# gafniguy/4D-Facial-Avatars

Measured on AMD Instinct MI355X. Metric: rays/sec at 512x512, 64 coarse + 128 fine samples, higher is better.
Workload: dtype f32; 1 GPU; configs[1]: paper-model eval forward, 512x512 frame, 64+128 samples, chunksize 65536, perturb on, expression+latent conditioned, background prior; frames sharded over GPUs

## Files before the change

### 4d-facial-avatars_amd/csrc/nf_mlp_gated.hip

```cpp
#include "nf_mlp_live_kernel.h"

__global__ void __launch_bounds__(256) k_paper_sigma_bound(const float* __restrict__ packed, float* __restrict__ bound) {
    using Net = NfPaperNet;
    __shared__ double sw[16][16], sv[16][16], sc[16], sd[16];
    __shared__ float fw[16], fv[16];
    const int tid = threadIdx.x, ni = blockIdx.x, part = tid >> 4, kk = tid & 15;
    auto alpha = [&](int n) { return (double)packed[Net::OFF_D0 + (((n >> 4) * 9 + 8) * 64 + ((n >> 2) & 3) * 16) * 4 + (n & 3)]; };
    double w = 0.0, v = 0.0, c = 0.0, d = 0.0;
    for (int j = 0; j < 16; ++j) {
        const int n = 16 * part + j;
        const double a = alpha(n);
        const double f = (double)packed[Net::OFF_FEAT + ((ni * 16 + (n >> 4)) * 64 + (kk >> 2) * 16 + (n & 15)) * 4 + (kk & 3)];
        w += a * f;
        v += fabs(a) * fabs(f);
        if (ni == 0 && kk == 0) {
            const double b = (double)packed[Net::OFF_BIAS + Net::B_FEAT + n];
            c += a * b;
            d += fabs(a) * fabs(b);
        }
    }
    sw[part][kk] = w;
    sv[part][kk] = v;
    if (kk == 0) {
        sc[part] = c;
        sd[part] = d;
    }
    __syncthreads();
    auto up = [](double x) {
        float f = (float)x;
        if ((double)f < x) f = nextafterf(f, INFINITY);
        return f;
    };
    if (tid < 16) {
        double tw = 0.0, tv = 0.0;
        for (int q = 0; q < 16; ++q) {
            tw += sw[q][tid];
            tv += sv[q][tid];
        }
        fw[tid] = (float)tw;
        fv[tid] = up(tv);
    }
    if (ni == 0 && tid == 16) {
        const double b = (double)packed[Net::OFF_BIAS + Net::B_D0 + 128];
        double tc = 0.0, td = 0.0;
        for (int q = 0; q < 16; ++q) {
            tc += sc[q];
            td += sd[q];
        }
        for (int j = 0; j < 16; ++j) bound[NF_BOUND_BIAS + j] = j == 0 ? (float)(tc + b) : (j == 1 ? up(td + fabs(b)) : 0.0f);
    }
    __syncthreads();
    const int lane = tid >> 2, r = tid & 3, g = lane >> 4, i = lane & 15;
    bound[(ni * 64 + lane) * 4 + r] = i == 0 ? fw[4 * g + r] : (i == 1 ? fv[4 * g + r] : 0.0f);
}

extern "C" size_t nf_paper_sigma_bound_floats(void) { return NF_BOUND_FLOATS; }

extern "C" int nf_paper_sigma_bound(const float* packed, float* bound, nf_stream_t stream) {
    if (!packed || !bound || ((uintptr_t)bound & 15)) return NF_EINVAL;
    hipLaunchKernelGGL(k_paper_sigma_bound, dim3(16), dim3(256), 0, nf_s(stream), packed, bound);
    NF_RETURN_LAUNCH();
}

extern "C" int nf_paper_mlp_fwd_gated(const float* packed, const float* bound, const float* cond, const float* ro, const float* rd,
                                      const float* rd_view, const float* z, int64_t n_rays, int n_samples, float* raw, float* scratch,
                                      size_t scratch_floats, int max_workgroups, nf_stream_t stream) {
    return nf_live_launch<false, true>(packed, cond, ro, rd, rd_view, z, n_rays, n_samples, raw, scratch, scratch_floats, max_workgroups, nullptr,
                                       stream, bound);
}
```

### 4d-facial-avatars_amd/csrc/nf_mlp_live_kernel.h

```cpp
#pragma once
#include <mutex>
#include "nf_mlp_paper_net.h"

#define NF_LIVE_ROWS 64
#ifndef NF_LIVE_PF
#define NF_LIVE_PF 8
#endif
#define NF_LIVE_DIR_B (NF_LIVE_ROWS * 1024)
#define NF_LIVE_META_B (NF_LIVE_DIR_B + NF_LIVE_ROWS * 64)
#define NF_LIVE_WAVE_B (NF_LIVE_META_B + NF_LIVE_ROWS * 16)
#define NF_LIVE_OOB NF_LIVE_WAVE_B
#define NF_LIVE_SC1 16

static_assert(NF_LIVE_ROWS == 64 && NF_MLP_NT == 2, "row numbers wrap with & 63; a pass's liveness is one 32-bit mask");
static_assert(NF_LIVE_PF >= 0 && NF_LIVE_PF <= 16, "prefetched rows live in registers beside fc_alpha's weights");

__device__ __forceinline__ __amdgpu_buffer_rsrc_t nf_live_ring(char* ring_v) {
    const uint64_t a = (uint64_t)ring_v;
    const uint64_t s = (uint64_t)(uint32_t)__builtin_amdgcn_readfirstlane((int)(uint32_t)a) |
                       ((uint64_t)(uint32_t)__builtin_amdgcn_readfirstlane((int)(a >> 32)) << 32);
    return __builtin_amdgcn_make_buffer_rsrc(reinterpret_cast<char*>(s), (short)0, NF_LIVE_WAVE_B, 0x00020000);
}
__device__ __forceinline__ void nf_live_store(__amdgpu_buffer_rsrc_t ring, int off_b, f32x4 v) {
    __builtin_amdgcn_raw_buffer_store_b128(__builtin_bit_cast(nf_u32x4, v), ring, off_b, 0, 0);
// ... 252 lines not shown
                    }
                }
                head_v = head + n_live;
                asm volatile("" : "+v"(head_v));
            }
            nf_live_mark<STATS, COLS>(stats, NF_LIVE_PH_APPEND, -1);
        } else {
            if constexpr (GATE) {
                NfGatePre pre{st, pf, ring_v, head_v, tail_v, bound_v};
                pre.wait();
                pre.loads(Wi, Ci, lane);
            } else {
                NfLivePre pre{st, wd, pf, ring_v, head_v, tail_v};
                pre.wait();
                pre.loads(Wi, Ci, lane);
            }
#pragma unroll
            for (int t = 0; t < NT; ++t) {
                dirf[t][0] = (f32x4){0.0f, 0.0f, 0.0f, 0.0f};
                sigma_own[t] = 0.0f;
            }
            run_v = __builtin_amdgcn_readfirstlane(head_v) != __builtin_amdgcn_readfirstlane(tail_v) ? 2 : 0;
        }
        asm volatile("" : "+v"(live_v), "+v"(run_v));
        const int run = __builtin_amdgcn_readfirstlane(run_v);
        if (run != 0) {
            nf_live_stat<STATS, COLS>(stats, NF_LIVE_STAT_RUNS, 1);
            if (run == 2) nf_live_stat<STATS, COLS>(stats, NF_LIVE_STAT_FLUSH, __builtin_amdgcn_readfirstlane(head_v) - __builtin_amdgcn_readfirstlane(tail_v));
            nf_live_mark<STATS, COLS>(stats, -1, NF_LIVE_PH_ENTRY);
            int lane_o = lane;
            asm volatile("" : "+v"(lane_o));
            const int g = lane_o >> 4, c = lane_o & 15;
            const __amdgpu_buffer_rsrc_t ring = nf_live_ring(ring_v);
            const int tail = __builtin_amdgcn_readfirstlane(tail_v), cnt = __builtin_amdgcn_readfirstlane(head_v) - tail;
            const unsigned own = run == 1 ? (unsigned)__builtin_amdgcn_readfirstlane(live_v) : 0u;
            const unsigned fill = run == 1 ? ~own : (1u << cnt) - 1u;
            const int n_fill = __builtin_popcount(fill);
            f32x4 meta[NT];
            bool valid[NT];
#pragma unroll
            for (int t = 0; t < NT; ++t) {
                const int bit = 16 * t + c;
                const bool f = (fill >> bit) & 1u;
                const int row = (tail + __builtin_popcount(fill & ((1u << bit) - 1u))) & (NF_LIVE_ROWS - 1);
                const f32x4 fd = nf_live_load(ring, f ? NF_LIVE_DIR_B + row * 64 + g * 16 : NF_LIVE_OOB);
                const f32x4 fm = nf_live_load(ring, f ? NF_LIVE_META_B + row * 16 : NF_LIVE_OOB);
                const int64_t p = (p0_v) + bit;
                dirf[t][0] = f ? fd : dirf[t][0];
                meta[t] = f ? fm : (f32x4){__int_as_float((int)(uint32_t)p), __int_as_float((int)(p >> 32)), GATE ? tag_own[t] : sigma_own[t], 0.0f};
                valid[t] = f || ((own >> bit) & 1u);
            }
            unsigned hh = fill;
#pragma unroll
            for (int i = 0; i < NF_LIVE_PF; ++i) {
                if (i < n_fill) {
                    const int h = nf_live_pop(hh);
                    act4[nf_live_slab(h, lane_o)] = pf[i];
                }
            }
#pragma unroll 1
            for (int i = NF_LIVE_PF; i < n_fill; i += 4) {
                f32x4 v[4];
                int h[4];
#pragma unroll
                for (int u = 0; u < 4; ++u) {
                    const bool ok = i + u < n_fill;
                    h[u] = ok ? nf_live_pop(hh) : -1;
                    v[u] = nf_live_load(ring, ok ? ((tail + i + u) & (NF_LIVE_ROWS - 1)) * 1024 + lane_o * 16 : NF_LIVE_OOB);
                }
#pragma unroll
                for (int u = 0; u < 4; ++u)
                    if (h[u] >= 0) act4[nf_live_slab(h[u], lane_o)] = v[u];
            }
            constexpr int NDIR = 1;
            constexpr unsigned D0 = Net::OFF_D0 / 4;
            nf_read_b<NT>(st.b0, act4, lane, 0);
            nf_live_mark<STATS, COLS>(stats, NF_LIVE_PH_ENTRY, NF_LIVE_PH_RUN);
            f32x4 acc[NT][16], bj[NT];
            float sigma_raw[NT];
            if constexpr (GATE) {
                nf_seg_lds<NT, 16, true, true>(acc, st, Wi, Net::OFF_FEAT / 4, 16, act4, lane);
                nf_pending_b<NT, true>(bj, st);
                nf_tail<NT, 16, 16, 9, 1>(acc, st.wb, bj, st, Wi, D0, Ci, Net::B_D0, act4, lane);
                NF_NET_COLOUR();
            } else {
                NF_NET_COLOUR_D0(8, 9, wd);
                NF_NET_COLOUR_REST();
            }
            int lane_s = lane;
            asm volatile("" : "+v"(lane_s));
            if ((lane_s >> 4) == 0) {
#pragma unroll
                for (int t = 0; t < NT; ++t) {
                    if (valid[t]) {
                        const int64_t p = (int64_t)(uint32_t)__float_as_int(meta[t].x) | ((int64_t)__float_as_int(meta[t].y) << 32);
                        if constexpr (GATE) {
                            const bool keep = !(sigma_raw[t] <= 0.0f) || __float_as_int(meta[t].z) != 0;
                            if (p >= 0 && p < n_points)
                                raw_v[p] = (f32x4){keep ? acc[t][0].x : 0.0f, keep ? acc[t][0].y : 0.0f, keep ? acc[t][0].z : 0.0f, sigma_raw[t]};
                        } else {
                            if (p >= 0 && p < n_points) raw_v[p] = (f32x4){acc[t][0].x, acc[t][0].y, acc[t][0].z, meta[t].z};
                        }
                    }
                }
            }
            tail_v = tail + n_fill;
            asm volatile("" : "+v"(tail_v));
            nf_live_mark<STATS, COLS>(stats, NF_LIVE_PH_RUN, -1);
        }
        asm volatile("" : "+v"(more_v));
        if (__builtin_amdgcn_readfirstlane(more_v) == 0) break;
        {
            nf_live_mark<STATS, COLS>(stats, -1, NF_LIVE_PH_DEAD);
            int lane_s = lane;
            asm volatile("" : "+v"(lane_s));
            const int g = lane_s >> 4, c = lane_s & 15;
            asm volatile("" : "+v"(live_v));
#pragma unroll
            for (int t = 0; t < NT; ++t) {
                const int64_t p = p0_v + 16 * t + c;
                if (g == 0 && p < n_points && !(((unsigned)live_v >> (16 * t + c)) & 1u)) raw_v[p] = (f32x4){0.0f, 0.0f, 0.0f, sigma_own[t]};
            }
            nf_live_mark<STATS, COLS>(stats, NF_LIVE_PH_DEAD, -1);
        }
        asm volatile("" : "+v"(next_v));
        unit_v = next_v;
    }
    nf_live_stat<STATS, COLS>(stats, NF_LIVE_STAT_CLOCK, (long long)wall_clock64(), true);
}

static inline int64_t nf_live_grid_cap(int max_workgroups) {
    const int64_t cu = nf_cu_count();
    return max_workgroups > 0 && max_workgroups < cu ? max_workgroups : cu;
}

#define NF_LIVE_SLOTS 256
#define NF_LIVE_SLOT_B 128

inline unsigned* nf_live_counter(hipStream_t stream) {
    struct Pool {
        char* base;
        const void* owner[NF_LIVE_SLOTS];
        int used;
    };
    static std::mutex mu;
    static Pool pools[64];
    static thread_local char this_thread;
    int dev = 0;
    if (hipGetDevice(&dev) != hipSuccess || dev < 0 || dev >= 64) return nullptr;
    const void* key = stream == hipStreamPerThread ? (const void*)&this_thread : (const void*)stream;
    std::lock_guard<std::mutex> lock(mu);
    Pool& p = pools[dev];
    if (!p.base) {
        void* mem = nullptr;
        if (hipMalloc(&mem, (size_t)NF_LIVE_SLOTS * NF_LIVE_SLOT_B) != hipSuccess) {
            (void)hipGetLastError();
            return nullptr;
        }
        p.base = (char*)mem;
        p.used = 0;
    }
    int i = 0;
    while (i < p.used && p.owner[i] != key) ++i;
    if (i == p.used) {
        if (p.used == NF_LIVE_SLOTS) {
            if (hipDeviceSynchronize() != hipSuccess) return nullptr;
            p.used = i = 0;
        }
        p.owner[p.used++] = key;
// ... 38 lines not shown
```

### 4d-facial-avatars_amd/csrc/nf_mlp_paper_net.h

```cpp
#pragma once
#include "nf_mlp_net_common.h"
#include "nf_mlp_smaller_layout.h"
#include "nf_pack.h"

#define NF_NET_COMMON(F)                                                                                                              \
    F(FRAG) F(NCOND) F(OFF_L0) F(OFF_L1) F(OFF_L2) F(OFF_L3) F(OFF_L4) F(OFF_FEAT) F(OFF_D0) F(OFF_D0E) F(OFF_D1) F(OFF_D2) F(OFF_RGB) \
    F(OFF_WC0) F(OFF_WC3) F(OFF_WCD) F(OFF_BIAS) F(B_L0) F(B_L1) F(B_L2) F(B_L3) F(B_L4) F(B_FEAT) F(B_D0) F(B_D1) F(B_D2) F(B_RGB)     \
    F(B_CVEC) F(B_DVEC) F(COND_FLOATS) F(S_PE) F(S_H0) F(S_H1) F(S_H2) F(S_H3) F(S_H4) F(S_FEAT) F(S_D0) F(S_D1) F(S_D2) F(S_DIRF)     \
    F(S_MASK) F(SAVED_PER_POINT) F(Z_L0) F(Z_L1) F(Z_L2) F(Z_L3) F(Z_L4) F(Z_FEAT) F(Z_D0) F(Z_D1) F(Z_D2) F(DZ_PER_POINT)             \
    F(OFFT_RGB) F(OFFT_D2) F(OFFT_D1) F(OFFT_D0) F(OFFT_FEAT) F(OFFT_L4) F(OFFT_L3) F(OFFT_L2) F(OFFT_L1)                              \
    F(G_L0) F(G_L1) F(G_L2) F(G_L3A) F(G_L3B) F(G_L4) F(G_FEAT) F(G_D0A) F(G_D0B) F(G_D1) F(G_D2) F(G_RGB) F(G_ALPHA)                  \
    F(CS_L0) F(CS_D0) F(CS_RGB) F(SLAB_FLOATS) F(GRAD_PARAM_FLOATS) F(GRAD_FLOATS)

struct NfPaperNet {
#define NF_NET_COPY(X) static constexpr int X = nfl::X;
    NF_NET_COMMON(NF_NET_COPY)
    NF_NET_COPY(OFF_L5) NF_NET_COPY(B_L5) NF_NET_COPY(S_H5) NF_NET_COPY(Z_L5) NF_NET_COPY(OFFT_L5) NF_NET_COPY(G_L5)
#undef NF_NET_COPY
    static constexpr bool HAS_L5 = true, D0_EXPR = false;
    static constexpr int PACKED = nfl::PACKED_FLOATS, PACKED_T = nfl::PACKED_T_FLOATS, NPARAMS = NF_PAPER_NUM_PARAMS;
    static constexpr int N_RELU = (nfl::SAVED_PER_POINT - nfl::S_MASK) / 8;
    static constexpr int D0_COLS = 280;
    static constexpr int MODEL = 0;
};
// ... 63 lines not shown
    for (int n = 0; n < 128; ++n) {
        for (int f = 0; f < 4; ++f)
            for (int sc = 0; sc < 2; ++sc)
                for (int comp = 1; comp < 3; ++comp)
                    t[Net::OFF_WCD + n * 16 + 4 * f + 2 * sc + (comp - 1)] = nf_code(id(NF_R_DIR0_W), n, 256 + 6 * f + 3 * sc + comp, Net::D0_COLS);
        if constexpr (Net::D0_EXPR)
            for (int k = 0; k < Net::NEXPR; ++k) t[Net::OFF_WCE + n * Net::NEXPR + k] = nf_code(id(NF_R_DIR0_W), n, 280 + k, Net::D0_COLS);
    }
    for (int n = 0; n < 256; ++n) {
        for (int l = 0; l < NX; ++l) t[Net::OFF_BIAS + 256 * l + n] = nf_code(2 * l + 1, 0, n, 256);
        t[Net::OFF_BIAS + Net::B_FEAT + n] = nf_code(id(NF_R_FEAT_B), 0, n, 256);
    }
    for (int n = 0; n < 128; ++n) {
        t[Net::OFF_BIAS + Net::B_D0 + n] = nf_code(id(NF_R_DIR0_B), 0, n, 128);
        t[Net::OFF_BIAS + Net::B_D1 + n] = nf_code(id(NF_R_DIR1_W) + 1, 0, n, 128);
        t[Net::OFF_BIAS + Net::B_D2 + n] = nf_code(id(NF_R_DIR2_W) + 1, 0, n, 128);
    }
    t[Net::OFF_BIAS + Net::B_D0 + 128] = nf_code(id(NF_R_ALPHA_B), 0, 0, 1);
    for (int n = 0; n < 3; ++n) t[Net::OFF_BIAS + Net::B_RGB + n] = nf_code(id(NF_R_RGB_B), 0, n, 3);
}

template <class Net>
static inline size_t nf_paper_net_saved_floats(int64_t n_points) {
    return (size_t)Net::SAVED_PER_POINT * (size_t)((n_points + 31) & ~(int64_t)31) + Net::N_RELU * 128;
}

template <class Net, bool DIRS>
__device__ __forceinline__ void nf_paper_net_condition(const float* __restrict__ packed, const float* __restrict__ expr,
                                                       const float* __restrict__ latent, float near_z, float far_z, float* __restrict__ cond) {
    __shared__ float cvec[Net::NCOND];
    __shared__ float dvec[16];
    const int tid = threadIdx.x;
    if (tid < 76) cvec[tid] = nf_div(nf_mul(expr[tid], 1.0f), 3.0f);
    else if (tid < Net::NCOND) cvec[tid] = latent[tid - 76];
    if (tid >= 128 && tid < 144) {
        const int k = tid - 128, f = k >> 2, sc = (k >> 1) & 1, comp = k & 1;
        const float a = nf_mul(comp ? far_z : near_z, exp2f((float)f));
        dvec[k] = DIRS ? (sc ? cosf(a) : sinf(a)) : 0.0f;
    }
    __syncthreads();
    const float* bias = packed + Net::OFF_BIAS;
    for (int i = blockIdx.x * blockDim.x + tid; i < Net::COND_FLOATS; i += gridDim.x * blockDim.x) {
        if (i >= Net::B_CVEC) { cond[i] = i < Net::B_DVEC ? cvec[i - Net::B_CVEC] : dvec[i - Net::B_DVEC]; continue; }
        float v = bias[i];
        if (i < Net::B_L1 || (i >= Net::B_L3 && i < Net::B_L4)) {
            const int n = i < Net::B_L1 ? i : i - Net::B_L3;
            const float* w = packed + (i < Net::B_L1 ? Net::OFF_WC0 : Net::OFF_WC3) + n * Net::NCOND;
            float s = 0.0f;
            for (int k = 0; k < Net::NCOND; ++k) s = fmaf(w[k], cvec[k], s);
            v += s;
        } else if ((DIRS || Net::D0_EXPR) && i >= Net::B_D0 && i < Net::B_D0 + 128) {
            float s = 0.0f;
            if (DIRS) {
                const float* w = packed + Net::OFF_WCD + (i - Net::B_D0) * 16;
                for (int k = 0; k < 16; ++k) s = fmaf(w[k], dvec[k], s);
            }
            if constexpr (Net::D0_EXPR) {
                const float* we = packed + Net::OFF_WCE + (i - Net::B_D0) * Net::NEXPR;
                for (int k = 0; k < Net::NEXPR; ++k) s = fmaf(we[k], cvec[k], s);
            }
            v += s;
        }
        cond[i] = v;
    }
}

template <class Net>
static inline dim3 nf_paper_net_condition_grid() { return dim3((Net::COND_FLOATS + 255) / 256); }

#define NF_NET_L3_PE()                                                                                        \
    do {                                                                                                      \
        NF_NET_PE_B(0); nf_chunk<NT, 16, true>(acc, st.wa, bj, st.bias);                                          \
        nf_load_w16<16>(st.wa, Wi, Net::OFF_L3 / 4 + 4 * 16 * 64, lane);    \
        nf_read_b<NT>(st.b0, act4, lane, 0);                                                                  \
        f32x4 w[16];                                                                                          \
        nf_load_w16<16>(w, Wi, Net::OFF_L3 / 4 + 1 * 16 * 64, lane);                                          \
        NF_NET_PE_B(1); nf_chunk<NT, 16, false>(acc, w, bj, st.bias);                                             \
        nf_load_w16<16>(w, Wi, Net::OFF_L3 / 4 + 2 * 16 * 64, lane);                                          \
        NF_NET_PE_B(2); nf_chunk<NT, 16, false>(acc, w, bj, st.bias);                                             \
        nf_load_w16<16>(w, Wi, Net::OFF_L3 / 4 + 3 * 16 * 64, lane);                                          \
        NF_NET_PE_B(3); nf_chunk<NT, 16, false>(acc, w, bj, st.bias);                                             \
    } while (0)

#define NF_NET_COLOUR_D0(NO0_, WS0_, WD_)                                                                                  \
                                \
    {                                                                                                                      \
        nf_seg_lds<NT, NO0_, true, false, WS0_>(acc, st, Wi, D0, 16, act4, lane);                                          \
        nf_pending_b<NT, false>(bj, st);                                                                                   \
        nf_chunk<NT, NO0_, false>(acc, st.wb, bj, st.bias);                                                                \
        if (NDIR == 2) {                                                                                                   \
            nf_load_w16<NO0_>(st.wb, Wi, D0 + 17 * (WS0_) * 64, lane);                                                     \
            _Pragma("unroll") for (int t = 0; t < NT; ++t) bj[t] = dirf[t][0];                                             \
            nf_chunk<NT, NO0_, false>(acc, WD_, bj, st.bias);                                                              \
        }                                                                                                                  \
        _Pragma("unroll") for (int t = 0; t < NT; ++t) bj[t] = dirf[t][NDIR - 1];                                          \
        if constexpr (NDIR == 2) nf_tail<NT, NO0_, 8, 8, 1>(acc, st.wb, bj, st, Wi, Net::OFF_D1 / 4, Ci, Net::B_D1, act4, lane); \
        else nf_tail<NT, NO0_, 8, 8, 1>(acc, WD_, bj, st, Wi, Net::OFF_D1 / 4, Ci, Net::B_D1, act4, lane);                  \
        if constexpr ((NO0_) > 8) { _Pragma("unroll") for (int t = 0; t < NT; ++t) sigma_raw[t] = acc[t][8].x; }           \
    }
#define NF_NET_COLOUR()                                                                                                    \
    {                                                                                                                      \
        f32x4 wd[16];                                                                                                      \
        nf_load_w16<9>(wd, Wi, D0 + 16 * 9 * 64, lane);                      \
        NF_NET_COLOUR_D0(9, 9, wd);                                                                                        \
    }                                                                                                                      \
    NF_NET_COLOUR_REST()
#define NF_NET_COLOUR_REST()                                                                                               \
                                                                                           \
    nf_seg_lds<NT, 8, true, true>(acc, st, Wi, Net::OFF_D1 / 4, 8, act4, lane);                                            \
    nf_pending_b<NT, true>(bj, st);                                                                                        \
    nf_tail<NT, 8, 8, 8, 1>(acc, st.wb, bj, st, Wi, Net::OFF_D2 / 4, Ci, Net::B_D2, act4, lane);                           \
    nf_seg_lds<NT, 8, true, true>(acc, st, Wi, Net::OFF_D2 / 4, 8, act4, lane);                                            \
    nf_pending_b<NT, true>(bj, st);                                                                                        \
    nf_tail<NT, 8, 8, 1, 1>(acc, st.wb, bj, st, Wi, Net::OFF_RGB / 4, Ci, Net::B_RGB, act4, lane);                         \
                                                                                                     \
    nf_seg_lds<NT, 1, true, true>(acc, st, Wi, Net::OFF_RGB / 4, 8, act4, lane);                                           \
    nf_pending_b<NT, true>(bj, st);                                                                                        \
    nf_chunk<NT, 1, false>(acc, st.wb, bj, st.bias)

struct NfNoPre {
    __device__ __forceinline__ void wait() const {}
    __device__ __forceinline__ void loads(const NfW&, const NfW&, int) const {}
};
#define NF_BOUND_BIAS 4096
#define NF_BOUND_FLOATS (NF_BOUND_BIAS + 16)
template <int NT, bool RELU_IN, class Pre>
__device__ __forceinline__ void nf_net_lone_tile(f32x4 (&acc)[NT][16], const NfStream<NT>& st, f32x4 (&bj)[NT], const NfW& W, unsigned first4,
                                                 unsigned stride4, const NfW& Wi, const NfW& Ci, const f32x4* act4, int lane, Pre& pre) {
    f32x4 w8[16];
    w8[0] = st.wa[0];
    pre.wait();
#pragma unroll
    for (int ch = 1; ch < 16; ++ch) w8[ch] = nf_load_w1(W, first4 + stride4 * ch, lane);
    if constexpr (RELU_IN) __builtin_amdgcn_sched_barrier(0);
    pre.loads(Wi, Ci, lane);
    if constexpr (RELU_IN) {
        f32x4 cur[NT], nxt[NT];
#pragma unroll
        for (int t = 0; t < NT; ++t) cur[t] = nf_relu_i(st.b0[t]);
#pragma unroll
        for (int ch = 0; ch < 16; ++ch) {
            if (ch + 1 < 16) nf_read_b<NT>(nxt, act4, lane, ch + 1);
            __builtin_amdgcn_sched_barrier(0);
#pragma unroll
            for (int r = 0; r < 2; ++r)
#pragma unroll
                for (int t = 0; t < NT; ++t)
                    acc[t][8] = __builtin_amdgcn_mfma_f32_16x16x4f32(w8[ch][r], cur[t][r], (ch == 0 && r == 0) ? st.bias[0] : acc[t][8], 0, 0, 0);
#pragma unroll
            for (int r = 2; r < 4; ++r)
#pragma unroll
                for (int t = 0; t < NT; ++t) {
                    __builtin_amdgcn_sched_barrier(0);
                    if (ch + 1 < 16) {
                        const int e = 2 * (r - 2);
#pragma unroll
                        for (int q = e; q < e + 2; ++q) {
                            const int xi = __float_as_int(nxt[t][q]);
                            nxt[t][q] = __int_as_float(xi > 0 ? xi : 0);
                        }
                    }
                    __builtin_amdgcn_sched_barrier(0);
                    acc[t][8] = __builtin_amdgcn_mfma_f32_16x16x4f32(w8[ch][r], cur[t][r], acc[t][8], 0, 0, 0);
                }
            __builtin_amdgcn_sched_barrier(0);
#pragma unroll
            for (int t = 0; t < NT; ++t) cur[t] = nxt[t];
        }
        return;
    }
#pragma unroll
    for (int ch = 0; ch < 16; ++ch) {
        if (ch == 0) {
#pragma unroll
            for (int t = 0; t < NT; ++t) bj[t] = RELU_IN ? nf_relu_i(st.b0[t]) : st.b0[t];
        } else {
            nf_read_b<NT>(bj, act4, lane, ch);
            if (RELU_IN) {
#pragma unroll
                for (int t = 0; t < NT; ++t) bj[t] = nf_relu_i(bj[t]);
            }
        }
#pragma unroll
        for (int r = 0; r < 4; ++r)
#pragma unroll
            for (int t = 0; t < NT; ++t)
                acc[t][8] = __builtin_amdgcn_mfma_f32_16x16x4f32(w8[ch][r], bj[t][r], (ch == 0 && r == 0) ? st.bias[0] : acc[t][8], 0, 0, 0);
    }
}
template <class Net, int NT, int NDIR, bool SIGMA = false, class Pre = NfNoPre, bool GATE = false>
__device__ __forceinline__ void nf_paper_net_body(f32x4 (&acc)[NT][16], float (&sigma_raw)[NT], const f32x4 (&pe)[NT][4],
                                                  const f32x4 (&dirf)[NT][NDIR], const NfW& Wi, const NfW& Ci, f32x4* act4, int lane,
                                                  Pre pre = Pre()) {
    static_assert(!GATE || (SIGMA && Net::HAS_L5), "the bound tile stands in for fc_alpha's lone tile, behind layers_xyz.5");
    constexpr unsigned D0 = (NDIR == 1 ? Net::OFF_D0 : Net::OFF_D0E) / 4;
    NfStream<NT> st;
    f32x4 bj[NT];
#define NF_NET_LAYER256(OFF_, FIRST_, OFF_NEXT_, B_NEXT_, NO_NEXT_, NEXT_B_)                                                \
    nf_seg_lds<NT, 16, FIRST_, true>(acc, st, Wi, OFF_, 16, act4, lane);                                                    \
    nf_pending_b<NT, true>(bj, st);                                                                                         \
    nf_tail<NT, 16, 16, NO_NEXT_, NEXT_B_>(acc, st.wb, bj, st, Wi, OFF_NEXT_, Ci, B_NEXT_, act4, lane)
    NF_NET_PE_LAYER(Net::B_L0, Net::OFF_L0, Net::OFF_L1, Net::B_L1);
    NF_NET_LAYER256(Net::OFF_L1 / 4, true, Net::OFF_L2 / 4, Net::B_L2, 16, 1);
    NF_NET_LAYER256(Net::OFF_L2 / 4, true, Net::OFF_L3 / 4, Net::B_L3, 16, 0);
    NF_NET_L3_PE();
    NF_NET_LAYER256(Net::OFF_L3 / 4 + 4 * 16 * 64, false, Net::OFF_L4 / 4, Net::B_L4, 16, 1);
    if constexpr (GATE) {
        NF_NET_LAYER256(Net::OFF_L4 / 4, true, Net::OFF_L5 / 4, Net::B_L5, 16, 1);
        const NfW Bi = pre.image();
        nf_seg_lds<NT, 16, true, true>(acc, st, Wi, Net::OFF_L5 / 4, 16, act4, lane);
        nf_pending_b<NT, true>(bj, st);
        nf_tail<NT, 16, 16, 1, 1>(acc, st.wb, bj, st, Bi, 0, Bi, NF_BOUND_BIAS, act4, lane);
        nf_net_lone_tile<NT, true>(acc, st, bj, Bi, 0, 64, Wi, Ci, act4, lane, pre);
        return;
    } else if constexpr (Net::HAS_L5) {
        NF_NET_LAYER256(Net::OFF_L4 / 4, true, Net::OFF_L5 / 4, Net::B_L5, 16, 1);
        NF_NET_LAYER256(Net::OFF_L5 / 4, true, Net::OFF_FEAT / 4, Net::B_FEAT, 16, 1);
    } else {
        NF_NET_LAYER256(Net::OFF_L4 / 4, true, Net::OFF_FEAT / 4, Net::B_FEAT, 16, 1);
    }
    if constexpr (SIGMA) {
        NF_NET_LAYER256(Net::OFF_FEAT / 4, true, D0 + 8 * 64, Net::B_D0 + 128, 1, 1);
        nf_net_lone_tile<NT, false>(acc, st, bj, Wi, D0 + 8 * 64, 9 * 64, Wi, Ci, act4, lane, pre);
#pragma unroll
        for (int t = 0; t < NT; ++t) sigma_raw[t] = acc[t][8].x;
        return;
    }
    NF_NET_LAYER256(Net::OFF_FEAT / 4, true, D0, Net::B_D0, 9, 1);
#undef NF_NET_LAYER256
    NF_NET_COLOUR();
}

template <class Net, int NT>
__device__ __forceinline__ void nf_paper_net_fwd_encoded(f32x4* lds, const float* __restrict__ packed, const float* __restrict__ cond,
                                                         const float* __restrict__ x87, int64_t n_points, float* __restrict__ out) {
    const int lane = threadIdx.x & 63, wave = threadIdx.x >> 6;
    const int64_t p0 = ((int64_t)blockIdx.x * NF_MLP_WAVES + wave) * (16 * NT);
    if (p0 >= n_points) return;
    f32x4* act4 = lds + wave * (16 * NT * 64);
    f32x4 pe[NT][4];
    f32x4 dirf[NT][2];
    nf_net_inputs_encoded<NT>(pe, dirf, p0, n_points, lane, x87);
    f32x4 acc[NT][16];
    float sigma_raw[NT];
    const NfW Wi = nf_w_image(packed, Net::PACKED), Ci = nf_w_image(cond, Net::COND_FLOATS);
    nf_paper_net_body<Net, NT, 2>(acc, sigma_raw, pe, dirf, Wi, Ci, act4, lane);
    nf_net_store_raw<NT>(acc, sigma_raw, p0, n_points, lane, out);
}

template <class Condition, class Forward>
static inline int nf_paper_net_forward_encoded(const float* packed, const float* x87, const float* expr76, const float* latent32,
                                               int64_t n_points, float* cond, float* out, Condition condition, Forward forward) {
    if (n_points == 0) return 0;
    if (!packed || !x87 || !expr76 || !latent32 || !cond || !out || n_points < 0) return NF_EINVAL;
    condition();
    const int64_t per_block = (int64_t)NF_MLP_WAVES * 16 * NF_MLP_NT;
    const int64_t grid = (n_points + per_block - 1) / per_block;
    if (grid > 0x7fffffff) return NF_EINVAL;
    forward((unsigned)grid);
    NF_RETURN_LAUNCH();
}

template <class Net, int NT>
__device__ __forceinline__ void nf_paper_net_body_save(f32x4 (&acc)[NT][16], float (&sigma_raw)[NT], const f32x4 (&pe)[NT][4],
                                                       const f32x4 (&dirf)[NT][1], const NfW& Wi, const NfW& Ci, f32x4* act4, int lane,
                                                       float* __restrict__ saved, int64_t p0, int64_t n) {
    static_assert(NT == 2, "the copy schedule below is written for 32-point slabs");
    constexpr int NX = nf_net_n_xyz<Net>;
    const int g = lane >> 4, c = lane & 15;
    auto sec = [&](int s, int width) { return nf_slab_copy(saved, s, width, p0, n); };
#pragma unroll
    for (int t = 0; t < NT; ++t) {
        const int64_t p = p0 + 16 * t + c;
        if (p < n) *reinterpret_cast<f32x4*>(saved + Net::S_DIRF * n + p * 16 + 4 * g) = dirf[t][0];
#pragma unroll
        for (int j = 0; j < 4; ++j) act4[nf_act_idx4(16 * t + c, 4 * j + g)] = pe[t][j];
    }
    {
        const NfSlabCopy cp = sec(Net::S_PE, 64);
#pragma unroll
        for (int k = 0; k < 16 * NT / 4; ++k) nf_copy_rows<16>(act4, cp, k, lane);
    }
    uint64_t m64[NT];
    NfStream<NT> st;
    f32x4 bj[NT];
#define NF_NET_LAYER128(OFF_, NO_, SEC_, MASKL_)                                                                          \
    NfCopyH<32, 4, true> cs{act4, sec(SEC_, 128), lane, 4, {}};                                                            \
    cs.prime();                                                                                                            \
    _Pragma("unroll") for (int t = 0; t < NT; ++t) m64[t] = 0;                                                             \
    nf_seg_lds<NT, NO_, true, true, true>(acc, st, Wi, OFF_, 8, act4, lane, cs, m64);                                      \
    NF_NET_SAVE_PENDING(true, MASKL_, 8)
    NF_NET_PE_LAYER(Net::B_L0, Net::OFF_L0, Net::OFF_L1, Net::B_L1);
    NF_NET_SAVE_LAYER256(Net::OFF_L1 / 4, true, Net::S_H0, 0, Net::OFF_L2 / 4, Net::B_L2, 16, 1);
    NF_NET_SAVE_LAYER256(Net::OFF_L2 / 4, true, Net::S_H1, 1, Net::OFF_L3 / 4, Net::B_L3, 16, 0);
    NF_NET_L3_PE();
    NF_NET_SAVE_LAYER256(Net::OFF_L3 / 4 + 4 * 16 * 64, false, Net::S_H2, 2, Net::OFF_L4 / 4, Net::B_L4, 16, 1);
    if constexpr (Net::HAS_L5) {
        NF_NET_SAVE_LAYER256(Net::OFF_L4 / 4, true, Net::S_H3, 3, Net::OFF_L5 / 4, Net::B_L5, 16, 1);
        NF_NET_SAVE_LAYER256(Net::OFF_L5 / 4, true, Net::S_H4, 4, Net::OFF_FEAT / 4, Net::B_FEAT, 16, 1);
        NF_NET_SAVE_LAYER256(Net::OFF_FEAT / 4, true, Net::S_H5, 5, Net::OFF_D0 / 4, Net::B_D0, 9, 1);
    } else {
        NF_NET_SAVE_LAYER256(Net::OFF_L4 / 4, true, Net::S_H3, 3, Net::OFF_FEAT / 4, Net::B_FEAT, 16, 1);
        NF_NET_SAVE_LAYER256(Net::OFF_FEAT / 4, true, Net::S_H4, 4, Net::OFF_D0 / 4, Net::B_D0, 9, 1);
    }
    {
        f32x4 wd[16];
        nf_load_w16<9>(wd, Wi, Net::OFF_D0 / 4 + 16 * 9 * 64, lane);
        NfCopyH<64, 4, false> cs{act4, sec(Net::S_FEAT, 256), lane, 8, {}};
        cs.prime();
        nf_seg_lds<NT, 9, true, false, false>(acc, st, Wi, Net::OFF_D0 / 4, 16, act4, lane, cs, m64);
        NF_NET_SAVE_PENDING(false, -1, 16);
        nf_chunk<NT, 9, false>(acc, st.wb, bj, st.bias);
#pragma unroll
// ... 108 lines not shown
```

### 4d-facial-avatars_amd/csrc/nf_mlp_stream.h

```cpp
#pragma once
#include "nf_mlp_dev.h"

#define NF_TAIL_LAG 2

template <int NT>
struct NfStream {
    f32x4 wa[16], wb[16];
    f32x4 bias[16];
    f32x4 b0[NT], b1[NT];
    f32x4 bp[NT];
};

__device__ __forceinline__ f32x4 nf_relu_i(f32x4 v) {
    f32x4 o;
#pragma unroll
    for (int r = 0; r < 4; ++r) {
        const int xi = __float_as_int(v[r]);
        o[r] = __int_as_float(xi > 0 ? xi : 0);
    }
    return o;
}

struct NfW {
    __amdgpu_buffer_rsrc_t rsrc;
// ... 79 lines not shown
    }
};

template <int NT>
__device__ __forceinline__ void nf_mask_bits(uint64_t (&m64)[NT], const f32x4 (&b)[NT], int ni) {
#pragma unroll
    for (int t = 0; t < NT; ++t) {
        uint32_t nib = 0u;
#pragma unroll
        for (int r = 0; r < 4; ++r) {
            const uint32_t y = (uint32_t)__float_as_int(b[t][r]);
            nib |= (y < 1u ? y : 1u) << r;
        }
        m64[t] |= (uint64_t)nib << (4 * ni);
    }
}

template <int NT, int NO, bool FIRST, bool RELU_IN, bool MASK, bool ST, bool RD, class Side>
__device__ __forceinline__ void nf_half(f32x4 (&acc)[NT][16], const f32x4 (&w)[16], const f32x4 (&raw)[NT], f32x4 (&wn)[16], f32x4 (&rawn)[NT],
                                        const f32x4 (&bias)[16], const NfW& W, unsigned wsrc, const f32x4* act4, int lane, int ni_next, Side& side,
                                        int step, uint64_t (&m64)[NT], f32x4 (&bp)[NT]) {
    constexpr int NS = ST ? Side::N : 0, NR = RD ? Side::N : 0;
    f32x4 b[NT];
#pragma unroll
    for (int t = 0; t < NT; ++t) b[t] = RELU_IN ? nf_relu_i(raw[t]) : raw[t];
    if (MASK && ST) {
        if (!RD) nf_mask_bits<NT>(m64, bp, ni_next - 2);
        nf_mask_bits<NT>(m64, b, ni_next - 1);
    }
    if (MASK && !ST) {
#pragma unroll
        for (int t = 0; t < NT; ++t) bp[t] = b[t];
    }
    nf_read_b<NT>(rawn, act4, lane, ni_next);
    const Side rows = side;
    if (RD) side.reads(step);
    nf_load_w16<NO>(wn, W, wsrc, lane);
    if (ST) rows.stores(step);
    nf_chunk<NT, NO, FIRST>(acc, w, b, bias);
    NF_SGB_N(0x100, NT + NR);
    if (RELU_IN) __builtin_amdgcn_sched_group_barrier(0x002, 4 * NT, 0);
#pragma unroll
    for (int no = 0; no < NO; ++no) {
        __builtin_amdgcn_sched_group_barrier(0x008, 4 * NT, 0);
        __builtin_amdgcn_sched_group_barrier(0x020, 1, 0);
        NF_SGB_N(0x040, (no + 1) * NS / NO - no * NS / NO);
    }
    __builtin_amdgcn_sched_barrier(0);
}

template <int NT, int NO, bool FIRST, bool RELU_IN, bool MASK, int WS = NO, class Side>
__device__ __forceinline__ void nf_seg_lds(f32x4 (&acc)[NT][16], NfStream<NT>& st, const NfW& W, unsigned wsec, int nch, const f32x4* act4,
                                           int lane, Side& side, uint64_t (&m64)[NT]) {
    static_assert(WS >= NO, "a chunk holds at least the tiles computed");
    if (MASK) {
#pragma unroll
        for (int t = 0; t < NT; ++t) st.bp[t] = (f32x4){0.f, 0.f, 0.f, 0.f};
    }
    __builtin_amdgcn_sched_barrier(0);
    nf_half<NT, NO, FIRST, RELU_IN, MASK, true, true>(acc, st.wa, st.b0, st.wb, st.b1, st.bias, W, wsec + WS * 64, act4, lane, 1, side, 0, m64, st.bp);
#pragma unroll 1
    for (int ni = 1; ni < nch - 1; ni += 2) {
        const int step = (ni + 1) >> 1;
        nf_half<NT, NO, false, RELU_IN, MASK, true, false>(acc, st.wb, st.b1, st.wa, st.b0, st.bias, W, wsec + (ni + 1) * WS * 64, act4, lane, ni + 1, side,
                                                           step, m64, st.bp);
        nf_half<NT, NO, false, RELU_IN, MASK, false, true>(acc, st.wa, st.b0, st.wb, st.b1, st.bias, W, wsec + (ni + 2) * WS * 64, act4, lane, ni + 2, side,
                                                           step, m64, st.bp);
    }
}
template <int NT, int NO, bool FIRST, bool RELU_IN, int WS = NO>
__device__ __forceinline__ void nf_seg_lds(f32x4 (&acc)[NT][16], NfStream<NT>& st, const NfW& W, unsigned wsec, int nch, const f32x4* act4,
                                           int lane) {
    NfNoCopy none;
    uint64_t unused[NT];
    nf_seg_lds<NT, NO, FIRST, RELU_IN, false, WS>(acc, st, W, wsec, nch, act4, lane, none, unused);
}

template <int NT, bool RELU_IN>
__device__ __forceinline__ void nf_pending_b(f32x4 (&b)[NT], const NfStream<NT>& st) {
#pragma unroll
    for (int t = 0; t < NT; ++t) b[t] = RELU_IN ? nf_relu_i(st.b1[t]) : st.b1[t];
}

template <int NT, int NO, int NO_ST, int NO_NEXT, int NEXT_B>
__device__ __forceinline__ void nf_tail(f32x4 (&acc)[NT][16], const f32x4 (&w)[16], const f32x4 (&b)[NT], NfStream<NT>& st,
                                        const NfW& W, unsigned wnext, const NfW& C, unsigned bias_next, f32x4* act4, int lane) {
    constexpr int LAG = NF_TAIL_LAG;
    constexpr int NL = 2 * NO_NEXT;
    const int g = lane >> 4, c = lane & 15;
    __builtin_amdgcn_sched_barrier(0);
    nf_load_bias<NO_NEXT>(st.bias, C, bias_next, lane);
    nf_load_w16<NO_NEXT>(st.wa, W, wnext, lane);
    f32x4 braw[NT];
#pragma unroll
    for (int no = 0; no < NO + LAG; ++no) {
        if (no < NO) {
#pragma unroll
            for (int r = 0; r < 4; ++r)
#pragma unroll
                for (int t = 0; t < NT; ++t) acc[t][no] = __builtin_amdgcn_mfma_f32_16x16x4f32(w[no][r], b[t][r], acc[t][no], 0, 0, 0);
        }
        if (no >= LAG && no - LAG < NO_ST) {
#pragma unroll
            for (int t = 0; t < NT; ++t) act4[nf_act_idx4(16 * t + c, 4 * (no - LAG) + g)] = acc[t][no - LAG];
        }
        if (no == LAG && NEXT_B != 0) {
#pragma unroll
            for (int t = 0; t < NT; ++t) braw[t] = act4[nf_act_idx4(16 * t + c, g)];
        }
    }
#pragma unroll
    for (int no = 0; no < NO + LAG; ++no) {
        if (no < NO) {
            __builtin_amdgcn_sched_group_barrier(0x008, 4 * NT, 0);
            NF_SGB_N(0x020, (no + 1) * NL / NO - no * NL / NO);
        }
        if (no >= LAG && no - LAG < NO_ST) __builtin_amdgcn_sched_group_barrier(0x200, NT, 0);
        if (no == LAG && NEXT_B != 0) __builtin_amdgcn_sched_group_barrier(0x100, NT, 0);
    }
    __builtin_amdgcn_sched_barrier(0);
    if (NEXT_B != 0) {
#pragma unroll
        for (int t = 0; t < NT; ++t) st.b0[t] = braw[t];
    }
}

template <int NT, int NO, int NO_NEXT, bool MASKED>
__device__ __forceinline__ void nf_tail_dz(f32x4 (&acc)[NT][16], const f32x4 (&w)[16], const f32x4 (&b)[NT], NfStream<NT>& st, const NfW& W,
                                           unsigned wnext, f32x4* act4, int lane, const uint2 (&m)[NT]) {
    constexpr int LAG = NF_TAIL_LAG;
    constexpr int NL = NO_NEXT;
    const int g = lane >> 4, c = lane & 15;
    __builtin_amdgcn_sched_barrier(0);
    if (NO_NEXT > 0) nf_load_w16<(NO_NEXT > 0 ? NO_NEXT : 1)>(st.wa, W, wnext, lane);
    f32x4 braw[NT];
#pragma unroll
    for (int no = 0; no < NO + LAG; ++no) {
        if (no < NO) {
#pragma unroll
            for (int r = 0; r < 4; ++r)
#pragma unroll
                for (int t = 0; t < NT; ++t) acc[t][no] = __builtin_amdgcn_mfma_f32_16x16x4f32(w[no][r], b[t][r], acc[t][no], 0, 0, 0);
        }
        if (no >= LAG) {
            const int q = no - LAG;
#pragma unroll
            for (int t = 0; t < NT; ++t) {
                f32x4 v = acc[t][q];
                if (MASKED) {
                    const uint32_t wd = q < 8 ? m[t].x : m[t].y;
#pragma unroll
                    for (int r = 0; r < 4; ++r) {
                        const int keep = ((int)(wd << (31 - (4 * (q & 7) + r)))) >> 31;
                        v[r] = __int_as_float(__float_as_int(v[r]) & keep);
                    }
                }
                act4[nf_act_idx4(16 * t + c, 4 * q + g)] = v;
            }
        }
        if (no == LAG && NO_NEXT > 0) {
#pragma unroll
            for (int t = 0; t < NT; ++t) braw[t] = act4[nf_act_idx4(16 * t + c, g)];
        }
    }
#pragma unroll
    for (int no = 0; no < NO + LAG; ++no) {
        if (no < NO) {
            __builtin_amdgcn_sched_group_barrier(0x008, 4 * NT, 0);
            NF_SGB_N(0x020, (no + 1) * NL / NO - no * NL / NO);
        }
        if (no >= LAG) {
            __builtin_amdgcn_sched_group_barrier(0x002, (MASKED ? 12 : 4) * NT, 0);
            __builtin_amdgcn_sched_group_barrier(0x200, NT, 0);
        }
        if (no == LAG && NO_NEXT > 0) __builtin_amdgcn_sched_group_barrier(0x100, NT, 0);
    }
    __builtin_amdgcn_sched_barrier(0);
    if (NO_NEXT > 0) {
#pragma unroll
        for (int t = 0; t < NT; ++t) st.b0[t] = braw[t];
    }
}
```

Before: 621,400 rays/s.

## Use 4x4 MFMA for sigma bound tile and trim colour tail K

Adds a dedicated bound tile that computes the sigma upper bound with 4x4x1 MFMAs into per-lane-group partials, reduced with permlane swaps, and prefetches activations two chunks ahead. This replaces the 16x16x4 lone-tile path that carried ReLU-in special casing. The bound packing is replicated across every fourth column, and the colour D0 tail in the gated kernel now runs only two of the four K sub-steps (NR=2), skipping MFMAs on direction inputs assumed zero-padded. It cuts MFMA work in the gating and colour paths, but relies on padding assumptions and adds cross-lane reduction cost.

```diff
diff --git a/4d-facial-avatars_amd/csrc/nf_mlp_gated.hip b/4d-facial-avatars_amd/csrc/nf_mlp_gated.hip
--- a/4d-facial-avatars_amd/csrc/nf_mlp_gated.hip
+++ b/4d-facial-avatars_amd/csrc/nf_mlp_gated.hip
@@ -51,7 +51,7 @@
     }
     __syncthreads();
     const int lane = tid >> 2, r = tid & 3, g = lane >> 4, i = lane & 15;
-    bound[(ni * 64 + lane) * 4 + r] = i == 0 ? fw[4 * g + r] : (i == 1 ? fv[4 * g + r] : 0.0f);
+    bound[(ni * 64 + lane) * 4 + r] = (i & 3) == 0 ? fw[4 * g + r] : ((i & 3) == 1 ? fv[4 * g + r] : 0.0f);
 }
 
 extern "C" size_t nf_paper_sigma_bound_floats(void) { return NF_BOUND_FLOATS; }
diff --git a/4d-facial-avatars_amd/csrc/nf_mlp_live_kernel.h b/4d-facial-avatars_amd/csrc/nf_mlp_live_kernel.h
--- a/4d-facial-avatars_amd/csrc/nf_mlp_live_kernel.h
+++ b/4d-facial-avatars_amd/csrc/nf_mlp_live_kernel.h
@@ -358,9 +358,9 @@
                 nf_seg_lds<NT, 16, true, true>(acc, st, Wi, Net::OFF_FEAT / 4, 16, act4, lane);
                 nf_pending_b<NT, true>(bj, st);
                 nf_tail<NT, 16, 16, 9, 1>(acc, st.wb, bj, st, Wi, D0, Ci, Net::B_D0, act4, lane);
-                NF_NET_COLOUR();
+                NF_NET_COLOUR(2);
             } else {
-                NF_NET_COLOUR_D0(8, 9, wd);
+                NF_NET_COLOUR_D0(8, 9, wd, 2);
                 NF_NET_COLOUR_REST();
             }
             int lane_s = lane;
diff --git a/4d-facial-avatars_amd/csrc/nf_mlp_paper_net.h b/4d-facial-avatars_amd/csrc/nf_mlp_paper_net.h
--- a/4d-facial-avatars_amd/csrc/nf_mlp_paper_net.h
+++ b/4d-facial-avatars_amd/csrc/nf_mlp_paper_net.h
@@ -169,7 +169,7 @@
         NF_NET_PE_B(3); nf_chunk<NT, 16, false>(acc, w, bj, st.bias);                                             \
     } while (0)
 
-#define NF_NET_COLOUR_D0(NO0_, WS0_, WD_)                                                                                  \
+#define NF_NET_COLOUR_D0(NO0_, WS0_, WD_, NR_)                                                                              \
                                 \
     {                                                                                                                      \
         nf_seg_lds<NT, NO0_, true, false, WS0_>(acc, st, Wi, D0, 16, act4, lane);                                          \
@@ -182,14 +182,14 @@
         }                                                                                                                  \
         _Pragma("unroll") for (int t = 0; t < NT; ++t) bj[t] = dirf[t][NDIR - 1];                                          \
         if constexpr (NDIR == 2) nf_tail<NT, NO0_, 8, 8, 1>(acc, st.wb, bj, st, Wi, Net::OFF_D1 / 4, Ci, Net::B_D1, act4, lane); \
-        else nf_tail<NT, NO0_, 8, 8, 1>(acc, WD_, bj, st, Wi, Net::OFF_D1 / 4, Ci, Net::B_D1, act4, lane);                  \
+        else nf_tail<NT, NO0_, 8, 8, 1, NR_>(acc, WD_, bj, st, Wi, Net::OFF_D1 / 4, Ci, Net::B_D1, act4, lane);             \
         if constexpr ((NO0_) > 8) { _Pragma("unroll") for (int t = 0; t < NT; ++t) sigma_raw[t] = acc[t][8].x; }           \
     }
-#define NF_NET_COLOUR()                                                                                                    \
+#define NF_NET_COLOUR(NR_)                                                                                                \
     {                                                                                                                      \
         f32x4 wd[16];                                                                                                      \
         nf_load_w16<9>(wd, Wi, D0 + 16 * 9 * 64, lane);                      \
-        NF_NET_COLOUR_D0(9, 9, wd);                                                                                        \
+        NF_NET_COLOUR_D0(9, 9, wd, NR_);                                                                                    \
     }                                                                                                                      \
     NF_NET_COLOUR_REST()
 #define NF_NET_COLOUR_REST()                                                                                               \
@@ -211,7 +211,7 @@
 };
 #define NF_BOUND_BIAS 4096
 #define NF_BOUND_FLOATS (NF_BOUND_BIAS + 16)
-template <int NT, bool RELU_IN, class Pre>
+template <int NT, class Pre>
 __device__ __forceinline__ void nf_net_lone_tile(f32x4 (&acc)[NT][16], const NfStream<NT>& st, f32x4 (&bj)[NT], const NfW& W, unsigned first4,
                                                  unsigned stride4, const NfW& Wi, const NfW& Ci, const f32x4* act4, int lane, Pre& pre) {
     f32x4 w8[16];
@@ -219,54 +219,14 @@
     pre.wait();
 #pragma unroll
     for (int ch = 1; ch < 16; ++ch) w8[ch] = nf_load_w1(W, first4 + stride4 * ch, lane);
-    if constexpr (RELU_IN) __builtin_amdgcn_sched_barrier(0);
     pre.loads(Wi, Ci, lane);
-    if constexpr (RELU_IN) {
-        f32x4 cur[NT], nxt[NT];
-#pragma unroll
-        for (int t = 0; t < NT; ++t) cur[t] = nf_relu_i(st.b0[t]);
-#pragma unroll
-        for (int ch = 0; ch < 16; ++ch) {
-            if (ch + 1 < 16) nf_read_b<NT>(nxt, act4, lane, ch + 1);
-            __builtin_amdgcn_sched_barrier(0);
-#pragma unroll
-            for (int r = 0; r < 2; ++r)
-#pragma unroll
-                for (int t = 0; t < NT; ++t)
-                    acc[t][8] = __builtin_amdgcn_mfma_f32_16x16x4f32(w8[ch][r], cur[t][r], (ch == 0 && r == 0) ? st.bias[0] : acc[t][8], 0, 0, 0);
-#pragma unroll
-            for (int r = 2; r < 4; ++r)
-#pragma unroll
-                for (int t = 0; t < NT; ++t) {
-                    __builtin_amdgcn_sched_barrier(0);
-                    if (ch + 1 < 16) {
-                        const int e = 2 * (r - 2);
-#pragma unroll
-                        for (int q = e; q < e + 2; ++q) {
-                            const int xi = __float_as_int(nxt[t][q]);
-                            nxt[t][q] = __int_as_float(xi > 0 ? xi : 0);
-                        }
-                    }
-                    __builtin_amdgcn_sched_barrier(0);
-                    acc[t][8] = __builtin_amdgcn_mfma_f32_16x16x4f32(w8[ch][r], cur[t][r], acc[t][8], 0, 0, 0);
-                }
-            __builtin_amdgcn_sched_barrier(0);
-#pragma unroll
-            for (int t = 0; t < NT; ++t) cur[t] = nxt[t];
-        }
-        return;
-    }
 #pragma unroll
     for (int ch = 0; ch < 16; ++ch) {
         if (ch == 0) {
 #pragma unroll
-            for (int t = 0; t < NT; ++t) bj[t] = RELU_IN ? nf_relu_i(st.b0[t]) : st.b0[t];
+            for (int t = 0; t < NT; ++t) bj[t] = st.b0[t];
         } else {
             nf_read_b<NT>(bj, act4, lane, ch);
-            if (RELU_IN) {
-#pragma unroll
-                for (int t = 0; t < NT; ++t) bj[t] = nf_relu_i(bj[t]);
-            }
         }
 #pragma unroll
         for (int r = 0; r < 4; ++r)
@@ -274,6 +234,50 @@
             for (int t = 0; t < NT; ++t)
                 acc[t][8] = __builtin_amdgcn_mfma_f32_16x16x4f32(w8[ch][r], bj[t][r], (ch == 0 && r == 0) ? st.bias[0] : acc[t][8], 0, 0, 0);
     }
+}
+__device__ __forceinline__ float nf_sum_lane_groups(float x) {
+    const auto a = __builtin_amdgcn_permlane32_swap(__float_as_uint(x), __float_as_uint(x), false, false);
+    const float y = nf_add(__uint_as_float(a[0]), __uint_as_float(a[1]));
+    const auto b = __builtin_amdgcn_permlane16_swap(__float_as_uint(y), __float_as_uint(y), false, false);
+    return nf_add(__uint_as_float(b[0]), __uint_as_float(b[1]));
+}
+template <int NT, class Pre>
+__device__ __forceinline__ void nf_net_bound_tile(f32x4 (&acc)[NT][16], const NfStream<NT>& st, const NfW& B, const NfW& Wi, const NfW& Ci,
+                                                  const f32x4* act4, int lane, Pre& pre) {
+    f32x4 w8[16], cur[NT], nxt[NT], far[NT], part[NT];
+    nf_read_b<NT>(nxt, act4, lane, 1);
+    w8[0] = st.wa[0];
+    pre.wait();
+#pragma unroll
+    for (int ch = 1; ch < 16; ++ch) w8[ch] = nf_load_w1(B, 64 * ch, lane);
+    __builtin_amdgcn_sched_barrier(0);
+    pre.loads(Wi, Ci, lane);
+#pragma unroll
+    for (int t = 0; t < NT; ++t) cur[t] = nf_relu_i(st.b0[t]);
+#pragma unroll
+    for (int ch = 0; ch < 16; ++ch) {
+        if (ch + 2 < 16) nf_read_b<NT>(far, act4, lane, ch + 2);
+#pragma unroll
+        for (int r = 0; r < 4; ++r)
+#pragma unroll
+            for (int t = 0; t < NT; ++t) {
+                __builtin_amdgcn_sched_barrier(0);
+                if (ch + 1 < 16) {
+                    const int xi = __float_as_int(nxt[t][r]);
+                    nxt[t][r] = __int_as_float(xi > 0 ? xi : 0);
+                }
+                __builtin_amdgcn_sched_barrier(0);
+                part[t] = __builtin_amdgcn_mfma_f32_4x4x1f32(w8[ch][r], cur[t][r], (ch == 0 && r == 0) ? st.bias[0] : part[t], 0, 0, 0);
+            }
+        __builtin_amdgcn_sched_barrier(0);
+#pragma unroll
+        for (int t = 0; t < NT; ++t) {
+            cur[t] = nxt[t];
+            nxt[t] = far[t];
+        }
+    }
+#pragma unroll
+    for (int t = 0; t < NT; ++t) acc[t][8] = (f32x4){nf_sum_lane_groups(part[t].x), nf_sum_lane_groups(part[t].y), 0.0f, 0.0f};
 }
 template <class Net, int NT, int NDIR, bool SIGMA = false, class Pre = NfNoPre, bool GATE = false>
 __device__ __forceinline__ void nf_paper_net_body(f32x4 (&acc)[NT][16], float (&sigma_raw)[NT], const f32x4 (&pe)[NT][4],
@@ -298,7 +302,7 @@
         nf_seg_lds<NT, 16, true, true>(acc, st, Wi, Net::OFF_L5 / 4, 16, act4, lane);
         nf_pending_b<NT, true>(bj, st);
         nf_tail<NT, 16, 16, 1, 1>(acc, st.wb, bj, st, Bi, 0, Bi, NF_BOUND_BIAS, act4, lane);
-        nf_net_lone_tile<NT, true>(acc, st, bj, Bi, 0, 64, Wi, Ci, act4, lane, pre);
+        nf_net_bound_tile<NT>(acc, st, Bi, Wi, Ci, act4, lane, pre);
         return;
     } else if constexpr (Net::HAS_L5) {
         NF_NET_LAYER256(Net::OFF_L4 / 4, true, Net::OFF_L5 / 4, Net::B_L5, 16, 1);
@@ -308,14 +312,14 @@
     }
     if constexpr (SIGMA) {
         NF_NET_LAYER256(Net::OFF_FEAT / 4, true, D0 + 8 * 64, Net::B_D0 + 128, 1, 1);
-        nf_net_lone_tile<NT, false>(acc, st, bj, Wi, D0 + 8 * 64, 9 * 64, Wi, Ci, act4, lane, pre);
+        nf_net_lone_tile<NT>(acc, st, bj, Wi, D0 + 8 * 64, 9 * 64, Wi, Ci, act4, lane, pre);
 #pragma unroll
         for (int t = 0; t < NT; ++t) sigma_raw[t] = acc[t][8].x;
         return;
     }
     NF_NET_LAYER256(Net::OFF_FEAT / 4, true, D0, Net::B_D0, 9, 1);
 #undef NF_NET_LAYER256
-    NF_NET_COLOUR();
+    NF_NET_COLOUR(4);
 }
 
 template <class Net, int NT>
diff --git a/4d-facial-avatars_amd/csrc/nf_mlp_stream.h b/4d-facial-avatars_amd/csrc/nf_mlp_stream.h
--- a/4d-facial-avatars_amd/csrc/nf_mlp_stream.h
+++ b/4d-facial-avatars_amd/csrc/nf_mlp_stream.h
@@ -185,7 +185,7 @@
     for (int t = 0; t < NT; ++t) b[t] = RELU_IN ? nf_relu_i(st.b1[t]) : st.b1[t];
 }
 
-template <int NT, int NO, int NO_ST, int NO_NEXT, int NEXT_B>
+template <int NT, int NO, int NO_ST, int NO_NEXT, int NEXT_B, int NR = 4>
 __device__ __forceinline__ void nf_tail(f32x4 (&acc)[NT][16], const f32x4 (&w)[16], const f32x4 (&b)[NT], NfStream<NT>& st,
                                         const NfW& W, unsigned wnext, const NfW& C, unsigned bias_next, f32x4* act4, int lane) {
     constexpr int LAG = NF_TAIL_LAG;
@@ -199,7 +199,7 @@
     for (int no = 0; no < NO + LAG; ++no) {
         if (no < NO) {
 #pragma unroll
-            for (int r = 0; r < 4; ++r)
+            for (int r = 0; r < NR; ++r)
 #pragma unroll
                 for (int t = 0; t < NT; ++t) acc[t][no] = __builtin_amdgcn_mfma_f32_16x16x4f32(w[no][r], b[t][r], acc[t][no], 0, 0, 0);
         }
@@ -215,7 +215,7 @@
 #pragma unroll
     for (int no = 0; no < NO + LAG; ++no) {
         if (no < NO) {
-            __builtin_amdgcn_sched_group_barrier(0x008, 4 * NT, 0);
+            __builtin_amdgcn_sched_group_barrier(0x008, NR * NT, 0);
             NF_SGB_N(0x020, (no + 1) * NL / NO - no * NL / NO);
         }
         if (no >= LAG && no - LAG < NO_ST) __builtin_amdgcn_sched_group_barrier(0x200, NT, 0);
```

Result: no change. 625,500 rays/s (median of 6 runs) (+0.7%).
